# mgokbulut/CG-RayTracer

Hardware: NVIDIA B200
Metric: Mrays/s (primary+shadow+bounce) (higher is better)
Workload: dtype f32

## Files before the change

cg-raytracer_b200/csrc/cgrt_capi.cu:

```cuda
#include "../../include/cgrt_b200.h"
#include "bvh_build.h"
#include "cgrt_kernels.h"

#include <algorithm>
#include <cfloat>
#include <climits>
#include <cmath>
#include <cstdio>
#include <cstring>
#include <map>
#include <mutex>
#include <string>
#include <vector>

using namespace cgrt;
#ifdef CGRT_INSTRUMENT
namespace cgrt { void readInstrumentation(unsigned long long* out, bool reset); void readTimeline(unsigned int* out, bool reset); void readStepHist(unsigned int* out, bool reset); }
#endif

static thread_local std::string g_err;
static int fail(int code, const std::string& msg)
{
    g_err = msg;
    return code;
// ... 1080 lines not shown
    T.recording = -1;
}

static bool waveTuning(WaveQ& Q, int nSlots, int nLights, int world)
{
    static int mode = 0, groupBelow = 400000, fin = 0, timeoutMs = 4000, switchBelow = 0, handOver = 1, tune = 1;
    static bool loaded = false;
    if (!loaded) {
        loaded = true;
        if (const char* e = getenv("CGRT_WAVE")) {
            std::string t(e);
            size_t pos = 0;
            while (pos < t.size()) {
                size_t c = t.find(',', pos);
                if (c == std::string::npos) c = t.size();
                const std::string kv = t.substr(pos, c - pos);
                const size_t eq = kv.find('=');
                if (eq != std::string::npos) {
                    const std::string key = kv.substr(0, eq);
                    const int v = atoi(kv.c_str() + eq + 1);
                    if (key == "mode") mode = v;
                    else if (key == "group_below") groupBelow = v;
                    else if (key == "fin") fin = v;
                    else if (key == "switch") switchBelow = v;
                    else if (key == "timeout_ms") timeoutMs = v;
                    else if (key == "handover") handOver = v;
                    else if (key == "tune") tune = v;
                }
                pos = c + 1;
            }
        }
    }
    Q.mode = mode == 1 || mode == 2 ? mode : (nSlots < groupBelow ? 2 : 1);
    Q.finEvery = fin > 0 ? std::max(fin, 2) : (nLights >= 3 ? 4 : (nLights == 2 ? 5 : (Q.mode == 2 && world > 1 ? 8 : 6)));
    Q.switchBelow = Q.mode == 2 ? 0 : (switchBelow > 0 ? switchBelow : (nSlots >= 1500000 ? 100000 : 60000));
    Q.timeoutNs = (unsigned long long)std::max(timeoutMs, 1) * 1000000ull;
    if (!handOver) Q.resume = nullptr;
    return fin <= 0 && tune != 0;
}

static int prepareFrame(cgrt_scene* s, const cgrt_camera* cams, int nViews, const cgrt_render_params* p, FrameParams& P,
                        const int** dTileList, const int2** dTileSeq, FramePipeline* pipe)
{
    const int tw = p->tile_w > 0 ? p->tile_w : 8, th = p->tile_h > 0 ? p->tile_h : 8;
    const int key[6] = {p->width, p->height, tw, th, p->world, p->rank};
    if (std::memcmp(key, s->tileKey, sizeof key) != 0 || !s->tileSeq.p) {
        TileLayout& L = s->layout;
        makeTileLayout(*p, L);
        const std::vector<int>& mine = L.lists[p->rank];
        std::vector<int2> seq(mine.size());
        std::vector<std::pair<float, int>> order(mine.size());
        s->primaryPixels = 0;
        for (size_t lt = 0; lt < mine.size(); lt++) {
            const int ty = mine[lt] / L.tilesX, tx = mine[lt] % L.tilesX;
            const float cx = (tx + 0.5f) * L.tileW - 0.5f * p->width, cy = (ty + 0.5f) * L.tileH - 0.5f * p->height;
            order[lt] = std::make_pair(cx * cx + cy * cy, (int)lt);
            const int w = std::min(L.tileW, p->width - tx * L.tileW), h = std::min(L.tileH, p->height - ty * L.tileH);
            s->primaryPixels += (uint64_t)w * h;
        }
        std::sort(order.begin(), order.end());
        for (size_t k = 0; k < order.size(); k++) seq[k] = make_int2(mine[order[k].second], order[k].second);
        RC(s->tileList.ensure(std::max<size_t>(mine.size(), 1)));
        RC(s->tileSeq.ensure(std::max<size_t>(mine.size(), 1)));
        CK(cudaDeviceSynchronize());
        if (!mine.empty()) {
            CK(cudaMemcpy(s->tileList.p, mine.data(), mine.size() * sizeof(int), cudaMemcpyHostToDevice));
            CK(cudaMemcpy(s->tileSeq.p, seq.data(), seq.size() * sizeof(int2), cudaMemcpyHostToDevice));
// ... 15 lines not shown
    P.tilesX = L.tilesX;
    P.world = L.world;
    P.rank = p->rank;
    P.screenLayout = (L.world == 1 || (p->flags & CGRT_RENDER_SCREEN_LAYOUT)) ? 1 : 0;
    const int64_t slots = (int64_t)nViews * (int64_t)L.lists[p->rank].size() * L.tileW * L.tileH;
    if (slots > INT_MAX) return fail(CGRT_ERR_INVALID, "too many pixel slots: views x tiles x tile pixels must stay below 2^31");
    P.nSlots = (int)slots;
    *dTileList = L.world > 1 ? s->tileList.p : nullptr;
    *dTileSeq = s->tileSeq.p;
    const size_t cap = (size_t)std::max(P.nSlots, 1);
    const int nL = std::max(P.nLights, 1);
    const int levels = std::max(P.traceLimit - 1, 1);
    const int pathLevels = std::max(P.traceLimit, 1);
    if (P.nSph > 0 && !useRounds(s, P)) return fail(CGRT_ERR_INVALID, "spherical lights need a scene with a search tree (not CGRT_SCENE_EXACT_ONLY / NO_SUBTREES)");
    *pipe = choosePipeline(s, P, p->flags);
    if (*pipe != PIPE_COUNT) {
        RC(s->hitRec.ensure(cap * pathLevels * 3));
        RC(s->pathDepth.ensure(cap));
        RC(s->lit.ensure(cap * pathLevels * nL));
    }
    switch (*pipe) {
    case PIPE_COUNT:
        RC(s->hitQ.ensure(cap * 3));
        RC(s->bounceQ.ensure(cap * 2));
        RC(s->lit.ensure(cap * nL));
        RC(s->pathState.ensure(cap * 2 * levels));
        break;
    case PIPE_WAVE: {
        const size_t tickets = waveTicketCap(P);
        if (tickets >= ((size_t)1 << 30)) return fail(CGRT_ERR_INVALID, "frame too large for the ray queue's 30-bit tickets");
        if (!s->waveRays.p || s->waveRays.n < tickets * 3) {
            RC(s->waveRays.ensure(tickets * 3));
            CK(cudaMemset(s->waveRays.p, 0, tickets * 3 * sizeof(float4)));
            RC(s->waveFin.ensure(tickets * 2));
            CK(cudaMemset(s->waveFin.p, 0, tickets * 2 * sizeof(float4)));
            CK(uploadsDone());
        }
        RC(s->waveCtl.ensure(WCTL_INTS));
        RC(s->waveResume.ensure((size_t)waveGridBlocks(s->di.numSMs) * 128 * WAVE_RESUME_F4));
        break;
    }
    case PIPE_ROUNDS: {
        if (P.nSph > 0) {
            RC(s->softList.ensure(cap * pathLevels + 1));
            RC(s->soft.ensure(cap * pathLevels * (size_t)P.nSph));
        }
        const size_t capR = cap + (size_t)CGRT_MAX_CHAINS * P.tileW * P.tileH;
        for (int k = 0; k < 2; k++) {
            RC(s->cRay[k].ensure(capR * 3));
            RC(s->cRes[k].ensure(capR));
            RC(s->sRay[k].ensure(capR * nL * 3));
            RC(s->sRes[k].ensure(capR * nL));
        }
        break;
    }
    case PIPE_PATHS:
        RC(s->hitList.ensure(cap * pathLevels));
        if (s->dev.fastRoot != 0u) {
            RC(s->replayQ.ensure(cap * 3));
            RC(s->replayShadow.ensure(cap * pathLevels * nL));
        }
        break;
    }
    RC(s->pathPix.ensure(cap));
    RC(s->counts.ensure(CGRT_CNT_TOTAL * CGRT_MAX_CHAINS));
    RC(s->tests.ensure(6));
    const size_t need = CGRT_PARAM_BLOCK_HEADER + ((size_t)nL + (size_t)P.nSph) * 32 + (size_t)nViews * CGRT_VIEW_F4 * 16;
    if (need > s->paramBlockBytes || !s->hParamRing) {
// ... 41 lines not shown
    B.replayQ = s->replayQ.p;
    B.replayShadow = s->replayShadow.p;
    B.counts = s->counts.p;
    B.cap = (size_t)std::max(P.nSlots, 1);
    B.levels = std::max(P.traceLimit, 1);
    return B;
}

static RoundBuffers roundBuffers(const cgrt_scene* s, const FrameParams& P, int c, int nChains)
{
    const size_t tpx = (size_t)P.tileW * P.tileH;
    const size_t capC = ((size_t)std::max(P.nSlots, 1) / tpx / nChains + 1) * tpx;
    const size_t nLc = (size_t)std::max(P.nLights, 1);
    RoundBuffers B;
    for (int k = 0; k < 2; k++) {
        B.cRay[k] = s->cRay[k].p + c * capC * 3; B.cRes[k] = s->cRes[k].p + c * capC;
        B.sRay[k] = s->sRay[k].p + c * capC * nLc * 3; B.sRes[k] = s->sRes[k].p + c * capC * nLc;
    }
    B.hitRec = s->hitRec.p;
    B.lit = s->lit.p;
    B.pathDepth = s->pathDepth.p;
    B.counts = s->counts.p + c * CGRT_CNT_TOTAL;
    B.levels = std::max(P.traceLimit, 1);
    B.softList = s->softList.p;
    B.soft = s->soft.p;
    B.softSeed = s->softSeed;
    return B;
}

static int waveQueues(cgrt_scene* s, cudaStream_t st, WaveQ& Q)
{
    Q.rays = s->waveRays.p;
    Q.fin = s->waveFin.p;
    Q.ctl = s->waveCtl.p;
    Q.seq = ++s->waveSeq;
    if (Q.seq == 0u) Q.seq = ++s->waveSeq;
    Q.cap = (int)std::min<size_t>(s->waveRays.n / 3, (size_t)0x3fffffff);
    Q.resume = s->waveResume.p;
    Q.resumeCap = (int)std::min<size_t>(s->waveResume.n / WAVE_RESUME_F4, (size_t)0xffffff);
    Q.lat = nullptr;
#ifdef CGRT_WAVE_LAT
    if (getenv("CGRT_WAVE_LAT")) {
        RC(s->waveLat.ensure((size_t)Q.cap * 16));
        CK(cudaMemsetAsync(s->waveLat.p, 0, (size_t)Q.cap * 16 * sizeof(unsigned), st));
        Q.lat = s->waveLat.p;
    }
#endif
    Q.trace = nullptr;
    if (getenv("CGRT_WAVE_TRACE") || Q.lat != nullptr) {
        RC(s->waveTrace.ensure((size_t)WAVE_TRACE_SAMPLES * 8));
        CK(cudaMemsetAsync(s->waveTrace.p, 0, (size_t)WAVE_TRACE_SAMPLES * 8 * sizeof(int), st));
        Q.trace = s->waveTrace.p;
    }
    return CGRT_OK;
}

static int renderDevice(cgrt_scene* s, const cgrt_camera* cams, int nViews, const cgrt_render_params* p, float* d_out, void* stream)
{
    RC(useSceneDevice(s));
    std::lock_guard<std::mutex> lk(s->mu);
    cudaStream_t st = (cudaStream_t)stream;
    FrameParams P;
    const int* dTiles = nullptr;
    const int2* dSeq = nullptr;
    FramePipeline pipe;
    RC(prepareFrame(s, cams, nViews, p, P, &dTiles, &dSeq, &pipe));
// ... 659 lines not shown
```

cg-raytracer_b200/csrc/cgrt_kernels.h:

```cpp
#pragma once
#include <cuda_runtime.h>
#include <stdint.h>
#include <stddef.h>

struct DevScene {
    const float4* nodes;
    const float4* triPl;
    const float4* triV0;
    const float4* triV1;
    const float4* triV2;
    const float4* tri4;
    const float4* tri4f;
    const float4* triN0;
    const float4* triN1;
    const float4* triN2;
    const float4* mats;
    const float4* spheres;
    const float4* pairs;
    const float4* wide;
    const float4* wide8;
    const int* origToLeaf;
    const int* alwaysTri;
    int nAlways;
    const int* refParent;
// ... 66 lines not shown
    int levels;
};

struct RoundBuffers {
    float4* cRay[2];
    float4* cRes[2];
    float4* sRay[2];
    float4* sRes[2];
    float4* hitRec;
    uint8_t* lit;
    int* pathDepth;
    int* counts;
    int levels;
    int* softList;
    float* soft;
    unsigned softSeed;
};

#define WCTL_PENDING 0
#define WCTL_ERR 2
#define WCTL_HEAD 32
#define WCTL_TAIL 64
#define WCTL_FHEAD 96
#define WCTL_FTAIL 128
#define WCTL_HEAD2 160
#define WCTL_TAIL2 192
#define WCTL_FINCOUNT 288
#define WCTL_FINEXIT 289
#define WCTL_T0 4
#define WCTL_CLOSEAT 224
#define WCTL_RESUME 256
#define WCTL_DONE 320
#define WCTL_SCRATCH (WCTL_DONE + 32 * 32)
#define WCTL_INTS (WCTL_SCRATCH + 32 * 32)

struct WaveQ {
    float4* rays;
    float4* fin;
    int* ctl;
    uint32_t seq;
    int cap;
    int mode;
    int switchBelow;
    int finEvery;
    unsigned long long timeoutNs;
    int resumeCap;
    float4* resume;
    unsigned* lat;
    int* trace;
};
#define WAVE_TRACE_SAMPLES 1024
#define WAVE_RESUME_STACK 32
#define WAVE_RESUME_F4 (1 + WAVE_RESUME_STACK / 2)

#define CGRT_TRACE_MAX_KERNELS (8 * (2 * (CGRT_MAX_LEVELS + 1) + 1) + 2)
struct WaveTrace {
    cudaEvent_t* ev;
    int maxKernels;
    int classMask;
    int n;
    int cls[CGRT_TRACE_MAX_KERNELS];
    int launches[4];
};

void launchSetupPlanes(const float4* v0, const float4* v1, const float4* v2, float4* pl, float4* tri4, int n, cudaStream_t st);
void launchPermuteTri4(const float4* tri4, const int* fastOrder, float4* tri4f, int n, cudaStream_t st);
void launchClosestBatch(const DevScene& S, const float4* rays, size_t n, float4* hits, uint32_t* counts, int numSMs,
                        cudaStream_t st);
void launchAnyBatch(const DevScene& S, const float4* rays, const float* maxDist, float eps, size_t n, uint8_t* occluded,
                    int numSMs, cudaStream_t st);
void launchBruteBatch(const DevScene& S, const float4* rays, size_t n, float4* hits, int numSMs, cudaStream_t st);
// ... 38 lines not shown
```

cg-raytracer_b200/csrc/cgrt_wave.cuh:

```cuda
#pragma once

#define WAVE_NSTAT 40
#define WAVE_STAT_PATHS 0
#define WAVE_STAT_HIT 1
#define WAVE_STAT_BOUNCE 17
#define WAVE_STAT_REPLAYC 35
#define WAVE_STAT_REPLAYS 36
struct WaveShared {
    int stat[WAVE_NSTAT];
    uint2 gstack[16][CGRT_STACK8];
};

enum { WS_NONE = 0, WS_WAIT = 1, WS_RUN = 2, WS_PASS = 3 };

RT_DEV unsigned ldRelaxedGpu(const unsigned* p)
{
    unsigned v;
    asm volatile("ld.relaxed.gpu.global.u32 %0, [%1];" : "=r"(v) : "l"(p) : "memory");
    return v;
}
RT_DEV void stRelaxedGpu(unsigned* p, unsigned v) { asm volatile("st.relaxed.gpu.global.u32 [%0], %1;" ::"l"(p), "r"(v) : "memory"); }
RT_DEV float4 ld128(const float4* p)
{
    unsigned long long lo, hi;
    asm volatile("{ .reg .b128 t; ld.relaxed.gpu.global.b128 t, [%2]; mov.b128 {%0, %1}, t; }" : "=l"(lo), "=l"(hi) : "l"(p) : "memory");
    return make_float4(__uint_as_float((unsigned)lo), __uint_as_float((unsigned)(lo >> 32)), __uint_as_float((unsigned)hi),
                       __uint_as_float((unsigned)(hi >> 32)));
}
RT_DEV void st128(float4* p, const float4& v)
{
    const unsigned long long lo = (unsigned long long)__float_as_uint(v.x) | ((unsigned long long)__float_as_uint(v.y) << 32);
    const unsigned long long hi = (unsigned long long)__float_as_uint(v.z) | ((unsigned long long)__float_as_uint(v.w) << 32);
    asm volatile("{ .reg .b128 t; mov.b128 t, {%1, %2}; st.relaxed.gpu.global.b128 [%0], t; }" ::"l"(p), "l"(lo), "l"(hi) : "memory");
}
RT_DEV void waveRelease(const WaveQ& Q)
{
    int* scratch = Q.ctl + WCTL_SCRATCH + 32 * ((blockIdx.x * 4 + (threadIdx.x >> 5)) & 31);
    asm volatile("red.release.gpu.global.add.u32 [%0], %1;" ::"l"(scratch), "r"(0) : "memory");
}
RT_DEV unsigned long long globalTimerNs()
{
    unsigned long long t;
    asm volatile("mov.u64 %0, %%globaltimer;" : "=l"(t));
    return t;
}
RT_DEV unsigned smId()
{
    unsigned v;
    asm("mov.u32 %0, %%smid;" : "=r"(v));
    return v;
}

#ifdef CGRT_WAVE_LAT
RT_DEV void waveLat(const WaveQ& Q, int tk, int k, unsigned v)
{
    if (Q.lat != nullptr && tk >= 0 && tk < Q.cap) Q.lat[16 * (size_t)tk + k] = v;
}
RT_DEV unsigned waveNow(const WaveQ& Q) { return (unsigned)globalTimerNs() - ldRelaxedGpu((const unsigned*)Q.ctl + WCTL_T0); }
#define WAVE_LAT(tk, k, v) waveLat(Q, tk, k, v)
#define WAVE_LAT_NOW(tk, k) waveLat(Q, tk, k, waveNow(Q))
#else
#define WAVE_LAT(tk, k, v)
#define WAVE_LAT_NOW(tk, k)
#endif

#define WAVE_SLOT_BITS 26
#define WAVE_CLOSED 0x40000000
#define WAVE_TAG2 0x80000000u
RT_DEV void waveStoreRay(const WaveQ& Q, int tk, unsigned tagBits, const V3& o, const V3& d, float bound, int meta)
{
    if (tk >= Q.cap) return;
    float4* q = Q.rays + 3 * (size_t)tk;
    const float tag = __uint_as_float(tagBits);
    st128(q, make_float4(o.x, o.y, o.z, tag));
    st128(q + 1, make_float4(d.x, d.y, d.z, tag));
    st128(q + 2, make_float4(bound, i2f(meta), 0.0f, tag));
    WAVE_LAT_NOW(tk, 0);
}
RT_DEV bool waveLoadRay(const WaveQ& Q, int tk, unsigned tagBits, float4& a, float4& b, float4& c)
{
    if (tk >= Q.cap) return false;
    const float4* r = Q.rays + 3 * (size_t)tk;
    a = ld128(r);
    b = ld128(r + 1);
    const float4 m = ld128(r + 2);
    const unsigned s = tagBits;
    const bool ok = __float_as_uint(a.w) == s && __float_as_uint(b.w) == s && __float_as_uint(m.w) == s;
    const int meta = f2i(m.y);
    if (meta & CGRT_RAY_ANY) {
        a.w = FLT_MAX;
        b.w = m.x;
        c = make_float4(0.0f, m.y, 0.001f, m.z);
    } else {
        a.w = m.x;
        b.w = __int_as_float(0x7f800000);
        c = make_float4(i2f(meta & ((1 << WAVE_SLOT_BITS) - 1)), i2f(meta >> WAVE_SLOT_BITS), 0.0f, m.z);
    }
    return ok;
}
RT_DEV bool wavePeekRay(const WaveQ& Q, bool mine, int tk, unsigned tagBits)
{
    const unsigned m = __ballot_sync(0xffffffffu, mine);
    if (m == 0u) return false;
    const int lowest = __reduce_min_sync(0xffffffffu, mine ? tk : 0x7fffffff);
    unsigned w = 0u;
    if ((threadIdx.x & 31) == 0 && lowest < Q.cap) w = ldRelaxedGpu((const unsigned*)(Q.rays + 3 * (size_t)lowest) + 11);
    return __shfl_sync(0xffffffffu, w, 0) == tagBits;
}
RT_DEV bool wavePeekFin(const WaveQ& Q, bool mine, int ftk)
{
    const unsigned m = __ballot_sync(0xffffffffu, mine);
    if (m == 0u) return false;
    const int lowest = __reduce_min_sync(0xffffffffu, mine ? ftk : 0x7fffffff);
    unsigned w = 0u;
    if ((threadIdx.x & 31) == 0 && lowest < Q.cap) w = ldRelaxedGpu((const unsigned*)(Q.fin + 2 * (size_t)lowest) + 7);
    return __shfl_sync(0xffffffffu, w, 0) == Q.seq;
}
RT_DEV int waveReserve(const WaveQ& Q, int n, bool& closedSeen, unsigned& tagBits)
{
    if (!closedSeen) {
        const int old = atomicAdd(Q.ctl + WCTL_TAIL, n);
        if (!(old & WAVE_CLOSED)) {
            tagBits = Q.seq;
            return old;
        }
        closedSeen = true;
    }
    const int t2 = atomicAdd(Q.ctl + WCTL_TAIL2, n);
    unsigned ca;
    while ((ca = ldRelaxedGpu((const unsigned*)Q.ctl + WCTL_CLOSEAT)) == 0u) { }
    tagBits = Q.seq | WAVE_TAG2;
    return (int)(ca - 1u) + t2;
}
RT_DEV int waveClaim(const WaveQ& Q, int headIdx, int n)
{
    int base = 0;
    if ((threadIdx.x & 31) == 0) base = atomicAdd(Q.ctl + headIdx, n);
    return __shfl_sync(0xffffffffu, base, 0);
}
RT_DEV void waveFinPush(const WaveQ& Q, bool mine, int tk, int state, float t, int tri, float t2)
{
    const unsigned mask = __ballot_sync(0xffffffffu, mine);
    if (mask == 0u) return;
    const int lane = threadIdx.x & 31, leader = __ffs(mask) - 1;
    int base = 0;
    if (lane == leader) base = atomicAdd(Q.ctl + WCTL_FTAIL, __popc(mask));
    base = __shfl_sync(0xffffffffu, base, leader);
    if (mine) {
        const int pos = base + __popc(mask & ((1u << lane) - 1u));
        if (pos < Q.cap) {
            const float tag = __uint_as_float(Q.seq);
            st128(Q.fin + 2 * (size_t)pos, make_float4(i2f(tk), i2f(state), t, tag));
            st128(Q.fin + 2 * (size_t)pos + 1, make_float4(i2f(tri), t2, tag, tag));
        }
    }
}
RT_DEV bool waveLoadFin(const WaveQ& Q, int ftk, int& tk, float4& res)
{
    if (ftk >= Q.cap) return false;
    const float4 c0 = ld128(Q.fin + 2 * (size_t)ftk), c1 = ld128(Q.fin + 2 * (size_t)ftk + 1);
    const unsigned s = Q.seq;
    tk = f2i(c0.x);
    res = make_float4(c0.y, c0.z, c1.x, c1.y);
    return __float_as_uint(c0.w) == s && __float_as_uint(c1.z) == s && __float_as_uint(c1.w) == s;
}
RT_DEV void waveRaiseDone(const WaveQ& Q)
{
    waveRelease(Q);
#pragma unroll 1
    for (int k = 0; k < 32; k++) stRelaxedGpu((unsigned*)Q.ctl + WCTL_DONE + 32 * k, 1u);
}
RT_DEV void wavePending(const WaveQ& Q, long long delta)
{
    unsigned long long* pend = (unsigned long long*)Q.ctl;
    const unsigned long long now = atomicAdd(pend, (unsigned long long)delta) + (unsigned long long)delta;
    if (now == ((unsigned long long)gridDim.x << 32)) {
        waveRaiseDone(Q);
    } else if (delta < 0 && Q.switchBelow > 0 && (now >> 32) == (unsigned long long)gridDim.x && (unsigned)now < (unsigned)Q.switchBelow) {
        if (ldRelaxedGpu((const unsigned*)Q.ctl + WCTL_CLOSEAT) == 0u) {
            const int old = atomicOr(Q.ctl + WCTL_TAIL, WAVE_CLOSED);
            if (!(old & WAVE_CLOSED)) stRelaxedGpu((unsigned*)Q.ctl + WCTL_CLOSEAT, (unsigned)old + 1u);
        }
    }
}
RT_DEV void wavePendingAdd(const WaveQ& Q, int created) { atomicAdd((unsigned long long*)Q.ctl, (unsigned long long)created); }
RT_DEV unsigned long long wavePendingIssue(const WaveQ& Q, long long delta)
{
    return atomicAdd((unsigned long long*)Q.ctl, (unsigned long long)delta) + (unsigned long long)delta;
}
RT_DEV void wavePendingCheck(const WaveQ& Q, unsigned long long now)
{
    if (now == ((unsigned long long)gridDim.x << 32)) {
        waveRaiseDone(Q);
// ... 4 lines not shown
        }
    }
}
RT_DEV bool waveDone(const WaveQ& Q)
{
    const int w = (blockIdx.x * 4 + (threadIdx.x >> 5)) & 31;
    unsigned f = 0u;
    if ((threadIdx.x & 31) == 0) f = ldRelaxedGpu((const unsigned*)Q.ctl + WCTL_DONE + 32 * w);
    return __shfl_sync(0xffffffffu, f, 0) != 0u;
}
#ifndef CGRT_WAVE_IDLE_MAX
#define CGRT_WAVE_IDLE_MAX 1000
#endif
RT_DEV void waveIdle(const WaveQ& Q, unsigned long long t0, int& idlePolls)
{
    __nanosleep(idlePolls < 8 ? 100 : (idlePolls < 32 ? 250 : (idlePolls < 128 ? 500 : CGRT_WAVE_IDLE_MAX)));
    if ((++idlePolls & 63) == 0 && (threadIdx.x & 31) == 0 && globalTimerNs() - t0 > Q.timeoutNs) {
        atomicExch(Q.ctl + WCTL_ERR, 1);
        waveRaiseDone(Q);
    }
}

RT_DEV void waveTraceSample(const WaveQ& Q, int& lastBucket)
{
    if (Q.trace == nullptr || (blockIdx.x & 15) != 0 || (threadIdx.x & 127) != 0) return;
    const unsigned t0 = ldRelaxedGpu((const unsigned*)Q.ctl + WCTL_T0);
    const int bucket = (int)(((unsigned)globalTimerNs() - t0) >> 12);
    if (bucket == lastBucket || bucket < 0 || bucket >= WAVE_TRACE_SAMPLES) return;
    lastBucket = bucket;
    int* o = Q.trace + 8 * bucket;
    o[1] = (int)ldRelaxedGpu((const unsigned*)Q.ctl + WCTL_PENDING);
    o[2] = (int)ldRelaxedGpu((const unsigned*)Q.ctl + WCTL_HEAD);
    o[3] = (int)ldRelaxedGpu((const unsigned*)Q.ctl + WCTL_TAIL);
    o[4] = (int)ldRelaxedGpu((const unsigned*)Q.ctl + WCTL_FHEAD);
    o[5] = (int)ldRelaxedGpu((const unsigned*)Q.ctl + WCTL_FTAIL);
    o[6] = (int)ldRelaxedGpu((const unsigned*)Q.ctl + WCTL_HEAD2);
    o[7] = (int)ldRelaxedGpu((const unsigned*)Q.ctl + WCTL_TAIL2);
    o[0] = 1;
}

#ifndef CGRT_WAVE_FIN_WAIT
#define CGRT_WAVE_FIN_WAIT 3
#endif
RT_DEV void waveFinishLoop(const DevScene& S, const FrameParams& P, const float4* __restrict__ lights, const WaveQ& Q,
                           const RoundBuffers& B, const int2* __restrict__ tileSeq, float* __restrict__ fb, WaveShared& sh,
                           unsigned long long t0)
{
    const int lane = threadIdx.x & 31;
    const unsigned ltMask = (1u << lane) - 1u;
    const int nL = P.nLights;
    int ftk = -1;
    int waited = 0, idlePolls = 0;
    bool closedSeen = false;
    int traceBucket = -1;
    int nextBase = 0, nextCount = 0;
    unsigned long long pendNow = 0ull;
    bool havePend = false, busy = false;
    {
        const int base = waveClaim(Q, WCTL_FHEAD, 32);
        ftk = base + lane;
    }
    while (true) {
        waveTraceSample(Q, traceBucket);
        if (nextCount) {
            const unsigned noneMask = __ballot_sync(0xffffffffu, ftk < 0);
            const int base = __shfl_sync(0xffffffffu, nextBase, 0);
            if (ftk < 0) ftk = base + __popc(noneMask & ltMask);
            nextCount = 0;
        }
        int tk = -1;
        float4 res = make_float4(0.0f, 0.0f, 0.0f, 0.0f);
        const bool ready = (busy || waited > 0 || wavePeekFin(Q, true, ftk)) && waveLoadFin(Q, ftk, tk, res);
        if (havePend) {
            wavePendingCheck(Q, pendNow);
            havePend = false;
        }
        const unsigned readyMask = __ballot_sync(0xffffffffu, ready);
        if (readyMask == 0u) {
            busy = false;
            if (waveDone(Q)) break;
            waveIdle(Q, t0, idlePolls);
            continue;
        }
        idlePolls = 0;
        if (readyMask != 0xffffffffu && busy && ++waited < CGRT_WAVE_FIN_WAIT) continue;
        busy = readyMask == 0xffffffffu && waited == 0;
        waited = 0;
        nextCount = __popc(readyMask);
        if (lane == 0) nextBase = atomicAdd(Q.ctl + WCTL_FHEAD, nextCount);
        const int n = __popc(readyMask);
        bool hit = false, bounce = false, replayC = false, replayS = false;
        V3 pointOn = mk3(0.0f, 0.0f, 0.0f), nn = pointOn, rd = pointOn;
        int slot = 0, rec = 0, level = 0;
        if (ready) {
            ftk = -1;
            float4 a, b, c;
            WAVE_LAT_NOW(tk, 4);
            waveLoadRay(Q, tk, 0u, a, b, c);
            const int meta = f2i(c.y);
#ifdef CGRT_WAVE_LAT
            if (a.x == 1e38f) return;
            WAVE_LAT_NOW(tk, 8);
#endif
            if (meta & CGRT_RAY_ANY) {
                const bool shadowed = finishShadowRay<true>(S, a, b, c, res, replayS);
                WAVE_LAT_NOW(tk, 9);
                B.lit[meta & 0x3fffffff] = shadowed ? 0 : 1;
            } else {
                const V3 o = mk3(a), d = mk3(b);
                slot = f2i(c.x);
                level = meta;
                TraceResult R;
                hit = finishClosestRay<true>(S, a, b, res, R, replayC);
#ifdef CGRT_WAVE_LAT
                if (R.t == -1e38f) return;
                WAVE_LAT_NOW(tk, 9);
#endif
                if (!hit) {
                    if (level == 0) {
                        int x, y, outIdx, local;
                        if (seqToPixel(P, tileSeq, slot, x, y, outIdx, local)) storeRGB(fb, outIdx, mk3(0.0f, 0.0f, 0.0f));
                    }
                } else {
                    int mat;
                    hitNormalAndMaterial(S, R, o, d, nn, mat);
                    pointOn = o + d * R.t;
                    rd = d;
                    rec = slot * B.levels + level;
                    float4* h = B.hitRec + 3 * (size_t)rec;
                    h[0] = make_float4(pointOn.x, pointOn.y, pointOn.z, i2f(mat));
                    h[1] = make_float4(nn.x, nn.y, nn.z, 0.0f);
                    h[2] = make_float4(d.x, d.y, d.z, 0.0f);
                    B.pathDepth[slot] = level + 1;
                    const float ksz = mat >= 0 ? __ldg(S.mats + 2 * mat + 1).z : 0.0f;
                    bounce = !(ksz <= 0.01f) && level + 1 < P.traceLimit;
                    atomicAdd(&sh.stat[WAVE_STAT_HIT + level], 1);
                    if (level == 0) atomicAdd(&sh.stat[WAVE_STAT_PATHS], 1);
                    if (bounce) atomicAdd(&sh.stat[WAVE_STAT_BOUNCE + level + 1], 1);
                    WAVE_LAT_NOW(tk, 10);
                }
                if (replayC) atomicAdd(&sh.stat[WAVE_STAT_REPLAYC], 1);
            }
            if (replayS) atomicAdd(&sh.stat[WAVE_STAT_REPLAYS], 1);
        }
        const int nShadow = hit ? nL : 0, nBounce = bounce ? 1 : 0;
        int sIncl = nShadow, bIncl = nBounce;
#pragma unroll
        for (int o = 1; o < 32; o <<= 1) {
            const int vs = __shfl_up_sync(0xffffffffu, sIncl, o), vb = __shfl_up_sync(0xffffffffu, bIncl, o);
            if (lane >= o) { sIncl += vs; bIncl += vb; }
        }
        const int totS = __shfl_sync(0xffffffffu, sIncl, 31), totB = __shfl_sync(0xffffffffu, bIncl, 31);
        int base = 0;
        unsigned tagBits = 0u;
        if (lane == 0 && totS + totB > 0) {
            wavePendingAdd(Q, totS + totB);
            base = waveReserve(Q, totS + totB, closedSeen, tagBits);
        }
        base = __shfl_sync(0xffffffffu, base, 0);
        tagBits = __shfl_sync(0xffffffffu, tagBits, 0);
        if (ready) WAVE_LAT_NOW(tk, 11);
        if (hit && nL > 0) {
            const int firstS = base + sIncl - nShadow;
            for (int l = 0; l < nL; l++) {
                V3 org, dir;
                float dist;
                shadowRayOf(lights, l, pointOn, org, dir, dist);
                waveStoreRay(Q, firstS + l, tagBits, org, dir, dist, CGRT_RAY_ANY | (rec * nL + l));
            }
        }
        if (bounce) {
            V3 org, dir;
            float tIn;
            reflectionRayOf(pointOn, rd, nn, org, dir, tIn);
            waveStoreRay(Q, base + totS + bIncl - 1, tagBits, org, dir, tIn, ((level + 1) << WAVE_SLOT_BITS) | slot);
        }
        if (ready) WAVE_LAT_NOW(tk, 5);
        if (lane == 0) {
            pendNow = wavePendingIssue(Q, -(long long)n);
            havePend = true;
        }
    }
    waveRelease(Q);
    __syncwarp();
    if (lane == 0) atomicAdd(Q.ctl + WCTL_FINEXIT, 1);
}

#ifndef CGRT_WAVE_STEPS
#define CGRT_WAVE_STEPS 8
#endif
#ifndef CGRT_WAVE_REFILL
#define CGRT_WAVE_REFILL 16
#endif
#ifndef CGRT_WAVE_GFIN
#define CGRT_WAVE_GFIN 1
#endif
#ifndef CGRT_WAVE_GSTEPS
#define CGRT_WAVE_GSTEPS 8
#endif
RT_DEV bool waveLaneLoop(const DevScene& S, const WaveQ& Q, unsigned long long t0)
{
    const int lane = threadIdx.x & 31;
    const unsigned ltMask = (1u << lane) - 1u;
    FastTrav T;
    FastStack K;
    int tk = -1, st = WS_NONE, state = TRAV_DONE;
    float eps = 0.0f, maxDist = 0.0f;
    bool any = false;
    int idlePolls = 0;
    int closeAt = 0x7fffffff;
    bool drained = false;
    T.t = 0.0f; T.hitTri = -1; T.node = 0u; T.sp = 0;
    K.t2 = 0.0f;
    while (true) {
        const bool fin = st == WS_RUN && state != TRAV_CONTINUE;
        const unsigned finMask = __ballot_sync(0xffffffffu, fin);
        const unsigned runMask = __ballot_sync(0xffffffffu, st == WS_RUN && !fin);
        const unsigned waitMask = __ballot_sync(0xffffffffu, st == WS_WAIT);
        const unsigned noneMask = __ballot_sync(0xffffffffu, st == WS_NONE || fin);
        const int nNone = __popc(noneMask), nFin = __popc(finMask);
        const bool open = closeAt == 0x7fffffff;
        const int want = (!drained && (!open || nNone >= CGRT_WAVE_REFILL || runMask == 0u) && nNone > 0) ? nNone : 0;
        int fbase = 0, base = 0;
        unsigned ca = 0u;
        if (lane == 0) {
            if (nFin) fbase = atomicAdd(Q.ctl + WCTL_FTAIL, nFin);
            if (want) base = atomicAdd(Q.ctl + WCTL_HEAD, want);
            if (open && Q.switchBelow > 0 && (waitMask != 0u || want != 0)) ca = ldRelaxedGpu((const unsigned*)Q.ctl + WCTL_CLOSEAT);
        }
        if (nFin) {
            fbase = __shfl_sync(0xffffffffu, fbase, 0);
            if (fin) {
                const int pos = fbase + __popc(finMask & ltMask);
                if (pos < Q.cap) {
                    const float tag = __uint_as_float(Q.seq);
                    st128(Q.fin + 2 * (size_t)pos, make_float4(i2f(tk), i2f(state), T.t, tag));
                    st128(Q.fin + 2 * (size_t)pos + 1, make_float4(i2f(T.hitTri), K.t2, tag, tag));
                }
                WAVE_LAT_NOW(tk, 3);
                st = WS_NONE;
                tk = -1;
            }
        }
        if (want) {
            base = __shfl_sync(0xffffffffu, base, 0);
            if (st == WS_NONE) {
                tk = base + __popc(noneMask & ltMask);
                st = WS_WAIT;
            }
        }
        if (open && Q.switchBelow > 0) {
            ca = __shfl_sync(0xffffffffu, ca, 0);
            if (ca != 0u) closeAt = (int)(ca - 1u);
        }
        const bool closed = closeAt != 0x7fffffff;
        if (closed && want != 0 && base + want > closeAt) drained = true;
        if (st == WS_WAIT && tk >= closeAt) { st = WS_NONE; tk = -1; }
        const bool handOver = closed && Q.resume != nullptr;
        if (handOver) {
            const bool mig = st == WS_RUN && state == TRAV_CONTINUE && T.sp <= WAVE_RESUME_STACK;
            const unsigned migMask = __ballot_sync(0xffffffffu, mig);
            if (migMask != 0u) {
                int rbase = 0, qbase = 0;
                if (lane == 0) {
                    rbase = atomicAdd(Q.ctl + WCTL_RESUME, __popc(migMask));
                    qbase = atomicAdd(Q.ctl + WCTL_TAIL2, __popc(migMask));
                }
                rbase = __shfl_sync(0xffffffffu, rbase, 0);
                qbase = __shfl_sync(0xffffffffu, qbase, 0);
                if (mig) {
                    const int r = rbase + __popc(migMask & ltMask), ntk = closeAt + qbase + __popc(migMask & ltMask);
// ... 69 lines not shown
            const bool run = st == WS_RUN && state == TRAV_CONTINUE;
            const bool leaf = run && travIsLeaf(T.node);
            const int sAll = __popc(__ballot_sync(0xffffffffu, run));
            const int sLeaf = __popc(__ballot_sync(0xffffffffu, leaf));
            const int nDone = __popc(__ballot_sync(0xffffffffu, st == WS_RUN && state != TRAV_CONTINUE));
            if (sAll == 0 || (nDone >= CGRT_WAVE_REFILL && it > 0)) break;
            if (sAll - sLeaf >= sLeaf) {
                if (run && !leaf) state = fastStepWideDyn(S, T, K, any, maxDist);
            } else {
                if (leaf) state = fastStepLeafDyn(S, T, K, any, eps, maxDist);
            }
        }
    }
}

RT_DEV void waveGroupLoop(const DevScene& S, const WaveQ& Q, WaveShared& sh, unsigned long long t0, int headIdx, int baseIdx,
                          unsigned tagBits)
{
    const int lane = threadIdx.x & 31, g = lane >> 3, j = lane & 7;
    uint2* K = sh.gstack[threadIdx.x >> 3];
    const float slack = 1.000001f;
    V3 o = mk3(0.0f, 0.0f, 0.0f), d = o, inv = o;
    float t = 0.0f, t2 = 0.0f, eps = 0.0f, maxDist = 0.0f;
    int hitTri = -1, tk = -1, st = WS_NONE, state = TRAV_DONE, sp = 0;
    uint32_t node = 0u;
    bool any = false;
    int idlePolls = 0;
#ifdef CGRT_WAVE_LAT
    int nsteps = 0;
#endif
    while (true) {
        const bool fin = st == WS_RUN && state != TRAV_CONTINUE;
        if (__any_sync(0xffffffffu, fin)) {
            waveFinPush(Q, fin && j == 0, tk, state, t, hitTri, t2);
#ifdef CGRT_WAVE_LAT
            if (fin && j == 0) { WAVE_LAT_NOW(tk, 3); WAVE_LAT(tk, 2, (unsigned)nsteps); }
#endif
            if (fin) { st = WS_NONE; tk = -1; }
        }
        const unsigned needy = __ballot_sync(0xffffffffu, st == WS_NONE && j == 0);
        if (needy != 0u) {
            const int base = waveClaim(Q, headIdx, __popc(needy));
            if (st == WS_NONE) {
                tk = baseIdx + base + __popc(needy & ((1u << (8 * g)) - 1u));
                st = WS_WAIT;
            }
        }
        const bool anyRun = __ballot_sync(0xffffffffu, st == WS_RUN) != 0u;
        if (anyRun ? __any_sync(0xffffffffu, st == WS_WAIT) : wavePeekRay(Q, st == WS_WAIT, tk, tagBits)) {
            float4 a = make_float4(0.0f, 0.0f, 0.0f, 0.0f), b = a, c = a;
            const bool rdy = st == WS_WAIT && waveLoadRay(Q, tk, tagBits, a, b, c);
            const unsigned rm = __ballot_sync(0xffffffffu, rdy);
            const bool start = ((rm >> (8 * g)) & 0xFFu) == 0xFFu;
            if (start) {
                o = mk3(a);
                d = mk3(b);
                maxDist = b.w;
                eps = c.z;
                any = (f2i(c.y) & CGRT_RAY_ANY) != 0;
                FastTrav T0;
                state = fastBegin(S, T0, o, d, a.w);
                inv = T0.inv;
                t = T0.t;
                t2 = __int_as_float(0x7f800000);
                hitTri = T0.hitTri;
                sp = 0;
                node = T0.node;
// ... 282 lines not shown
```

Before: 2641.

## Split wave finish queue into separate closest-hit and shadow queues

Finished traversal records now go into two queues, one for closest-hit rays and one for shadow (any-hit) rays, each with its own head and tail counters. A single 64-bit atomic reserves slots in both at once. The finisher warps consume homogeneous batches from one queue at a time, so shadow and closest-hit shading no longer diverge within a warp. The change also alters the default finEvery for mode 1 with one light, and doubles the finish-buffer size.

```diff
diff --git a/cg-raytracer_b200/csrc/cgrt_capi.cu b/cg-raytracer_b200/csrc/cgrt_capi.cu
--- a/cg-raytracer_b200/csrc/cgrt_capi.cu
+++ b/cg-raytracer_b200/csrc/cgrt_capi.cu
@@ -1136,7 +1136,7 @@
         }
     }
     Q.mode = mode == 1 || mode == 2 ? mode : (nSlots < groupBelow ? 2 : 1);
-    Q.finEvery = fin > 0 ? std::max(fin, 2) : (nLights >= 3 ? 4 : (nLights == 2 ? 5 : (Q.mode == 2 && world > 1 ? 8 : 6)));
+    Q.finEvery = fin > 0 ? std::max(fin, 2) : (nLights >= 3 ? 4 : (nLights == 2 ? 5 : (Q.mode == 2 ? (world > 1 ? 8 : 6) : 7)));
     Q.switchBelow = Q.mode == 2 ? 0 : (switchBelow > 0 ? switchBelow : (nSlots >= 1500000 ? 100000 : 60000));
     Q.timeoutNs = (unsigned long long)std::max(timeoutMs, 1) * 1000000ull;
     if (!handOver) Q.resume = nullptr;
@@ -1218,8 +1218,8 @@
         if (!s->waveRays.p || s->waveRays.n < tickets * 3) {
             RC(s->waveRays.ensure(tickets * 3));
             CK(cudaMemset(s->waveRays.p, 0, tickets * 3 * sizeof(float4)));
-            RC(s->waveFin.ensure(tickets * 2));
-            CK(cudaMemset(s->waveFin.p, 0, tickets * 2 * sizeof(float4)));
+            RC(s->waveFin.ensure(tickets * 4));
+            CK(cudaMemset(s->waveFin.p, 0, tickets * 4 * sizeof(float4)));
             CK(uploadsDone());
         }
         RC(s->waveCtl.ensure(WCTL_INTS));
@@ -1327,6 +1327,7 @@
 {
     Q.rays = s->waveRays.p;
     Q.fin = s->waveFin.p;
+    Q.sfin = s->waveFin.p + s->waveFin.n / 2;
     Q.ctl = s->waveCtl.p;
     Q.seq = ++s->waveSeq;
     if (Q.seq == 0u) Q.seq = ++s->waveSeq;
diff --git a/cg-raytracer_b200/csrc/cgrt_kernels.h b/cg-raytracer_b200/csrc/cgrt_kernels.h
--- a/cg-raytracer_b200/csrc/cgrt_kernels.h
+++ b/cg-raytracer_b200/csrc/cgrt_kernels.h
@@ -122,11 +122,14 @@
 #define WCTL_RESUME 256
 #define WCTL_DONE 320
 #define WCTL_SCRATCH (WCTL_DONE + 32 * 32)
-#define WCTL_INTS (WCTL_SCRATCH + 32 * 32)
+#define WCTL_SFHEAD (WCTL_SCRATCH + 32 * 32)
+#define WCTL_SFTAIL (WCTL_FTAIL + 1)
+#define WCTL_INTS (WCTL_SFHEAD + 32)
 
 struct WaveQ {
     float4* rays;
     float4* fin;
+    float4* sfin;
     int* ctl;
     uint32_t seq;
     int cap;
diff --git a/cg-raytracer_b200/csrc/cgrt_wave.cuh b/cg-raytracer_b200/csrc/cgrt_wave.cuh
--- a/cg-raytracer_b200/csrc/cgrt_wave.cuh
+++ b/cg-raytracer_b200/csrc/cgrt_wave.cuh
@@ -52,6 +52,11 @@
 }
 
 #ifdef CGRT_WAVE_LAT
+#define WAVE_LAT_CLOSEST_HIT 1u
+#define WAVE_LAT_CLOSEST_MISS 2u
+#define WAVE_LAT_SHADOW_FIRED 3u
+#define WAVE_LAT_SHADOW_DONE 4u
+#define WAVE_LAT_REPLAY 8u
 RT_DEV void waveLat(const WaveQ& Q, int tk, int k, unsigned v)
 {
     if (Q.lat != nullptr && tk >= 0 && tk < Q.cap) Q.lat[16 * (size_t)tk + k] = v;
@@ -107,14 +112,16 @@
     if ((threadIdx.x & 31) == 0 && lowest < Q.cap) w = ldRelaxedGpu((const unsigned*)(Q.rays + 3 * (size_t)lowest) + 11);
     return __shfl_sync(0xffffffffu, w, 0) == tagBits;
 }
-RT_DEV bool wavePeekFin(const WaveQ& Q, bool mine, int ftk)
-{
-    const unsigned m = __ballot_sync(0xffffffffu, mine);
-    if (m == 0u) return false;
-    const int lowest = __reduce_min_sync(0xffffffffu, mine ? ftk : 0x7fffffff);
-    unsigned w = 0u;
-    if ((threadIdx.x & 31) == 0 && lowest < Q.cap) w = ldRelaxedGpu((const unsigned*)(Q.fin + 2 * (size_t)lowest) + 7);
-    return __shfl_sync(0xffffffffu, w, 0) == Q.seq;
+RT_DEV void wavePeekFin(const WaveQ& Q, int ftkC, int ftkS, bool& servedC, bool& servedS)
+{
+    const int lowC = __reduce_min_sync(0xffffffffu, ftkC), lowS = __reduce_min_sync(0xffffffffu, ftkS);
+    unsigned wc = 0u, ws = 0u;
+    if ((threadIdx.x & 31) == 0) {
+        if (lowC < Q.cap) wc = ldRelaxedGpu((const unsigned*)(Q.fin + 2 * (size_t)lowC) + 7);
+        if (lowS < Q.cap) ws = ldRelaxedGpu((const unsigned*)(Q.sfin + 2 * (size_t)lowS) + 7);
+    }
+    servedC = __shfl_sync(0xffffffffu, wc, 0) == Q.seq;
+    servedS = __shfl_sync(0xffffffffu, ws, 0) == Q.seq;
 }
 RT_DEV int waveReserve(const WaveQ& Q, int n, bool& closedSeen, unsigned& tagBits)
 {
@@ -138,27 +145,34 @@
     if ((threadIdx.x & 31) == 0) base = atomicAdd(Q.ctl + headIdx, n);
     return __shfl_sync(0xffffffffu, base, 0);
 }
-RT_DEV void waveFinPush(const WaveQ& Q, bool mine, int tk, int state, float t, int tri, float t2)
+RT_DEV void waveFinStore(const WaveQ& Q, bool any, int pos, int tk, int state, float t, int tri, float t2)
+{
+    if (pos >= Q.cap) return;
+    float4* f = (any ? Q.sfin : Q.fin) + 2 * (size_t)pos;
+    const float tag = __uint_as_float(Q.seq);
+    st128(f, make_float4(i2f(tk), i2f(state), t, tag));
+    st128(f + 1, make_float4(i2f(tri), t2, tag, tag));
+}
+RT_DEV unsigned long long waveFinReserve(const WaveQ& Q, unsigned cMask, unsigned sMask)
+{
+    return atomicAdd((unsigned long long*)(Q.ctl + WCTL_FTAIL), (unsigned long long)__popc(cMask) | ((unsigned long long)__popc(sMask) << 32));
+}
+RT_DEV void waveFinPush(const WaveQ& Q, bool mine, bool any, int tk, int state, float t, int tri, float t2)
 {
     const unsigned mask = __ballot_sync(0xffffffffu, mine);
     if (mask == 0u) return;
+    const unsigned sMask = __ballot_sync(0xffffffffu, mine && any), cMask = mask & ~sMask;
     const int lane = threadIdx.x & 31, leader = __ffs(mask) - 1;
-    int base = 0;
-    if (lane == leader) base = atomicAdd(Q.ctl + WCTL_FTAIL, __popc(mask));
-    base = __shfl_sync(0xffffffffu, base, leader);
-    if (mine) {
-        const int pos = base + __popc(mask & ((1u << lane) - 1u));
-        if (pos < Q.cap) {
-            const float tag = __uint_as_float(Q.seq);
-            st128(Q.fin + 2 * (size_t)pos, make_float4(i2f(tk), i2f(state), t, tag));
-            st128(Q.fin + 2 * (size_t)pos + 1, make_float4(i2f(tri), t2, tag, tag));
-        }
-    }
-}
-RT_DEV bool waveLoadFin(const WaveQ& Q, int ftk, int& tk, float4& res)
+    unsigned long long bases = 0ull;
+    if (lane == leader) bases = waveFinReserve(Q, cMask, sMask);
+    bases = __shfl_sync(0xffffffffu, bases, leader);
+    if (mine) waveFinStore(Q, any, (int)(any ? (unsigned)(bases >> 32) : (unsigned)bases) + __popc((any ? sMask : cMask) & ((1u << lane) - 1u)), tk, state, t, tri, t2);
+}
+RT_DEV bool waveLoadFin(const WaveQ& Q, bool any, int ftk, int& tk, float4& res)
 {
     if (ftk >= Q.cap) return false;
-    const float4 c0 = ld128(Q.fin + 2 * (size_t)ftk), c1 = ld128(Q.fin + 2 * (size_t)ftk + 1);
+    const float4* f = (any ? Q.sfin : Q.fin) + 2 * (size_t)ftk;
+    const float4 c0 = ld128(f), c1 = ld128(f + 1);
     const unsigned s = Q.seq;
     tk = f2i(c0.x);
     res = make_float4(c0.y, c0.z, c1.x, c1.y);
@@ -229,8 +243,8 @@
     o[1] = (int)ldRelaxedGpu((const unsigned*)Q.ctl + WCTL_PENDING);
     o[2] = (int)ldRelaxedGpu((const unsigned*)Q.ctl + WCTL_HEAD);
     o[3] = (int)ldRelaxedGpu((const unsigned*)Q.ctl + WCTL_TAIL);
-    o[4] = (int)ldRelaxedGpu((const unsigned*)Q.ctl + WCTL_FHEAD);
-    o[5] = (int)ldRelaxedGpu((const unsigned*)Q.ctl + WCTL_FTAIL);
+    o[4] = (int)(ldRelaxedGpu((const unsigned*)Q.ctl + WCTL_FHEAD) + ldRelaxedGpu((const unsigned*)Q.ctl + WCTL_SFHEAD));
+    o[5] = (int)(ldRelaxedGpu((const unsigned*)Q.ctl + WCTL_FTAIL) + ldRelaxedGpu((const unsigned*)Q.ctl + WCTL_SFTAIL));
     o[6] = (int)ldRelaxedGpu((const unsigned*)Q.ctl + WCTL_HEAD2);
     o[7] = (int)ldRelaxedGpu((const unsigned*)Q.ctl + WCTL_TAIL2);
     o[0] = 1;
@@ -246,72 +260,124 @@
     const int lane = threadIdx.x & 31;
     const unsigned ltMask = (1u << lane) - 1u;
     const int nL = P.nLights;
-    int ftk = -1;
-    int waited = 0, idlePolls = 0;
+    int ftkC = -1, ftkS = -1;
+    int waitedC = 0, waitedS = 0, idlePolls = 0;
     bool closedSeen = false;
     int traceBucket = -1;
     int nextBase = 0, nextCount = 0;
+    bool lastShadow = false;
     unsigned long long pendNow = 0ull;
-    bool havePend = false, busy = false;
+    bool havePend = false, busyC = false, busyS = false;
     {
-        const int base = waveClaim(Q, WCTL_FHEAD, 32);
-        ftk = base + lane;
+        int baseC = 0, baseS = 0;
+        if (lane == 0) {
+            baseC = atomicAdd(Q.ctl + WCTL_FHEAD, 32);
+            baseS = atomicAdd(Q.ctl + WCTL_SFHEAD, 32);
+        }
+        ftkC = __shfl_sync(0xffffffffu, baseC, 0) + lane;
+        ftkS = __shfl_sync(0xffffffffu, baseS, 0) + lane;
     }
     while (true) {
         waveTraceSample(Q, traceBucket);
         if (nextCount) {
-            const unsigned noneMask = __ballot_sync(0xffffffffu, ftk < 0);
+            const bool none = (lastShadow ? ftkS : ftkC) < 0;
+            const unsigned noneMask = __ballot_sync(0xffffffffu, none);
             const int base = __shfl_sync(0xffffffffu, nextBase, 0);
-            if (ftk < 0) ftk = base + __popc(noneMask & ltMask);
+            if (none) {
+                if (lastShadow) ftkS = base + __popc(noneMask & ltMask);
+                else ftkC = base + __popc(noneMask & ltMask);
+            }
             nextCount = 0;
         }
-        int tk = -1;
-        float4 res = make_float4(0.0f, 0.0f, 0.0f, 0.0f);
-        const bool ready = (busy || waited > 0 || wavePeekFin(Q, true, ftk)) && waveLoadFin(Q, ftk, tk, res);
+        bool lookC = busyC || waitedC > 0, lookS = busyS || waitedS > 0;
+        if (!lookC || !lookS) {
+            bool servedC, servedS;
+            wavePeekFin(Q, ftkC, ftkS, servedC, servedS);
+            lookC = lookC || servedC;
+            lookS = lookS || servedS;
+        }
+        int tkC = -1, tkS = -1;
+        float4 resC = make_float4(0.0f, 0.0f, 0.0f, 0.0f), resS = resC;
+        const bool readyC = lookC && waveLoadFin(Q, false, ftkC, tkC, resC);
+        const bool readyS = lookS && waveLoadFin(Q, true, ftkS, tkS, resS);
         if (havePend) {
             wavePendingCheck(Q, pendNow);
             havePend = false;
         }
-        const unsigned readyMask = __ballot_sync(0xffffffffu, ready);
-        if (readyMask == 0u) {
-            busy = false;
+        const unsigned maskC = __ballot_sync(0xffffffffu, readyC), maskS = __ballot_sync(0xffffffffu, readyS);
+        if (maskC == 0u) busyC = false;
+        if (maskS == 0u) busyS = false;
+        if ((maskC | maskS) == 0u) {
             if (waveDone(Q)) break;
             waveIdle(Q, t0, idlePolls);
             continue;
         }
         idlePolls = 0;
-        if (readyMask != 0xffffffffu && busy && ++waited < CGRT_WAVE_FIN_WAIT) continue;
-        busy = readyMask == 0xffffffffu && waited == 0;
-        waited = 0;
+        const bool goC = maskC != 0u && (maskC == 0xffffffffu || !busyC || ++waitedC >= CGRT_WAVE_FIN_WAIT);
+        const bool goS = maskS != 0u && (maskS == 0xffffffffu || !busyS || ++waitedS >= CGRT_WAVE_FIN_WAIT);
+        if (!goC && !goS) continue;
+        const bool shadowBatch = goS && !goC;
+        lastShadow = shadowBatch;
+        const unsigned readyMask = shadowBatch ? maskS : maskC;
+        if (shadowBatch) {
+            busyS = maskS == 0xffffffffu && waitedS == 0;
+            waitedS = 0;
+        } else {
+            busyC = maskC == 0xffffffffu && waitedC == 0;
+            waitedC = 0;
+        }
         nextCount = __popc(readyMask);
-        if (lane == 0) nextBase = atomicAdd(Q.ctl + WCTL_FHEAD, nextCount);
-        const int n = __popc(readyMask);
-        bool hit = false, bounce = false, replayC = false, replayS = false;
-        V3 pointOn = mk3(0.0f, 0.0f, 0.0f), nn = pointOn, rd = pointOn;
-        int slot = 0, rec = 0, level = 0;
-        if (ready) {
-            ftk = -1;
-            float4 a, b, c;
-            WAVE_LAT_NOW(tk, 4);
-            waveLoadRay(Q, tk, 0u, a, b, c);
-            const int meta = f2i(c.y);
-#ifdef CGRT_WAVE_LAT
-            if (a.x == 1e38f) return;
-            WAVE_LAT_NOW(tk, 8);
-#endif
-            if (meta & CGRT_RAY_ANY) {
-                const bool shadowed = finishShadowRay<true>(S, a, b, c, res, replayS);
-                WAVE_LAT_NOW(tk, 9);
+        if (lane == 0) nextBase = atomicAdd(Q.ctl + (shadowBatch ? WCTL_SFHEAD : WCTL_FHEAD), nextCount);
+        const int n = nextCount;
+#ifdef CGRT_WAVE_LAT
+        const unsigned latB0 = __shfl_sync(0xffffffffu, waveNow(Q), 0);
+        unsigned latCls = 0u;
+        const int tk = shadowBatch ? tkS : tkC;
+        const bool ready = shadowBatch ? readyS : readyC;
+#endif
+        if (shadowBatch) {
+            if (readyS) {
+                ftkS = -1;
+                float4 a, b, c;
+                bool replayS = false;
+                WAVE_LAT_NOW(tkS, 4);
+                waveLoadRay(Q, tkS, 0u, a, b, c);
+                const int meta = f2i(c.y);
+#ifdef CGRT_WAVE_LAT
+                if (a.x == 1e38f) return;
+                WAVE_LAT_NOW(tkS, 8);
+#endif
+                const bool shadowed = finishShadowRay<true>(S, a, b, c, resS, replayS);
+                WAVE_LAT_NOW(tkS, 9);
                 B.lit[meta & 0x3fffffff] = shadowed ? 0 : 1;
-            } else {
+#ifdef CGRT_WAVE_LAT
+                latCls = (f2i(resS.x) == TRAV_FIRED ? WAVE_LAT_SHADOW_FIRED : WAVE_LAT_SHADOW_DONE) | (replayS ? WAVE_LAT_REPLAY : 0u);
+#endif
+                if (replayS) atomicAdd(&sh.stat[WAVE_STAT_REPLAYS], 1);
+                WAVE_LAT_NOW(tkS, 11);
+                WAVE_LAT_NOW(tkS, 5);
+            }
+        } else {
+            bool hit = false, bounce = false, replayC = false;
+            V3 pointOn = mk3(0.0f, 0.0f, 0.0f), nn = pointOn, rd = pointOn;
+            int slot = 0, rec = 0, level = 0;
+            if (readyC) {
+                ftkC = -1;
+                float4 a, b, c;
+                WAVE_LAT_NOW(tkC, 4);
+                waveLoadRay(Q, tkC, 0u, a, b, c);
+#ifdef CGRT_WAVE_LAT
+                if (a.x == 1e38f) return;
+                WAVE_LAT_NOW(tkC, 8);
+#endif
                 const V3 o = mk3(a), d = mk3(b);
                 slot = f2i(c.x);
-                level = meta;
+                level = f2i(c.y);
                 TraceResult R;
-                hit = finishClosestRay<true>(S, a, b, res, R, replayC);
+                hit = finishClosestRay<true>(S, a, b, resC, R, replayC);
 #ifdef CGRT_WAVE_LAT
                 if (R.t == -1e38f) return;
-                WAVE_LAT_NOW(tk, 9);
+                WAVE_LAT_NOW(tkC, 9);
 #endif
                 if (!hit) {
                     if (level == 0) {
@@ -334,45 +400,51 @@
                     atomicAdd(&sh.stat[WAVE_STAT_HIT + level], 1);
                     if (level == 0) atomicAdd(&sh.stat[WAVE_STAT_PATHS], 1);
                     if (bounce) atomicAdd(&sh.stat[WAVE_STAT_BOUNCE + level + 1], 1);
-                    WAVE_LAT_NOW(tk, 10);
+                    WAVE_LAT_NOW(tkC, 10);
                 }
                 if (replayC) atomicAdd(&sh.stat[WAVE_STAT_REPLAYC], 1);
-            }
-            if (replayS) atomicAdd(&sh.stat[WAVE_STAT_REPLAYS], 1);
-        }
-        const int nShadow = hit ? nL : 0, nBounce = bounce ? 1 : 0;
-        int sIncl = nShadow, bIncl = nBounce;
+#ifdef CGRT_WAVE_LAT
+                latCls = (hit ? WAVE_LAT_CLOSEST_HIT : WAVE_LAT_CLOSEST_MISS) | (replayC ? WAVE_LAT_REPLAY : 0u);
+#endif
+            }
+            const int nShadow = hit ? nL : 0, nBounce = bounce ? 1 : 0;
+            int sIncl = nShadow, bIncl = nBounce;
 #pragma unroll
-        for (int o = 1; o < 32; o <<= 1) {
-            const int vs = __shfl_up_sync(0xffffffffu, sIncl, o), vb = __shfl_up_sync(0xffffffffu, bIncl, o);
-            if (lane >= o) { sIncl += vs; bIncl += vb; }
-        }
-        const int totS = __shfl_sync(0xffffffffu, sIncl, 31), totB = __shfl_sync(0xffffffffu, bIncl, 31);
-        int base = 0;
-        unsigned tagBits = 0u;
-        if (lane == 0 && totS + totB > 0) {
-            wavePendingAdd(Q, totS + totB);
-            base = waveReserve(Q, totS + totB, closedSeen, tagBits);
-        }
-        base = __shfl_sync(0xffffffffu, base, 0);
-        tagBits = __shfl_sync(0xffffffffu, tagBits, 0);
-        if (ready) WAVE_LAT_NOW(tk, 11);
-        if (hit && nL > 0) {
-            const int firstS = base + sIncl - nShadow;
-            for (int l = 0; l < nL; l++) {
+            for (int o = 1; o < 32; o <<= 1) {
+                const int vs = __shfl_up_sync(0xffffffffu, sIncl, o), vb = __shfl_up_sync(0xffffffffu, bIncl, o);
+                if (lane >= o) { sIncl += vs; bIncl += vb; }
+            }
+            const int totS = __shfl_sync(0xffffffffu, sIncl, 31), totB = __shfl_sync(0xffffffffu, bIncl, 31);
+            int base = 0;
+            unsigned tagBits = 0u;
+            if (lane == 0 && totS + totB > 0) {
+                wavePendingAdd(Q, totS + totB);
+                base = waveReserve(Q, totS + totB, closedSeen, tagBits);
+            }
+            base = __shfl_sync(0xffffffffu, base, 0);
+            tagBits = __shfl_sync(0xffffffffu, tagBits, 0);
+            if (readyC) WAVE_LAT_NOW(tkC, 11);
+            if (hit && nL > 0) {
+                const int firstS = base + sIncl - nShadow;
+                for (int l = 0; l < nL; l++) {
+                    V3 org, dir;
+                    float dist;
+                    shadowRayOf(lights, l, pointOn, org, dir, dist);
+                    waveStoreRay(Q, firstS + l, tagBits, org, dir, dist, CGRT_RAY_ANY | (rec * nL + l));
+                }
+            }
+            if (bounce) {
                 V3 org, dir;
-                float dist;
-                shadowRayOf(lights, l, pointOn, org, dir, dist);
-                waveStoreRay(Q, firstS + l, tagBits, org, dir, dist, CGRT_RAY_ANY | (rec * nL + l));
-            }
-        }
-        if (bounce) {
-            V3 org, dir;
-            float tIn;
-            reflectionRayOf(pointOn, rd, nn, org, dir, tIn);
-            waveStoreRay(Q, base + totS + bIncl - 1, tagBits, org, dir, tIn, ((level + 1) << WAVE_SLOT_BITS) | slot);
-        }
-        if (ready) WAVE_LAT_NOW(tk, 5);
+                float tIn;
+                reflectionRayOf(pointOn, rd, nn, org, dir, tIn);
+                waveStoreRay(Q, base + totS + bIncl - 1, tagBits, org, dir, tIn, ((level + 1) << WAVE_SLOT_BITS) | slot);
+            }
+            if (readyC) WAVE_LAT_NOW(tkC, 5);
+        }
+#ifdef CGRT_WAVE_LAT
+        const unsigned latB1 = __shfl_sync(0xffffffffu, waveNow(Q), 0);
+        if (ready) { WAVE_LAT(tk, 12, latB0); WAVE_LAT(tk, 13, latB1); WAVE_LAT(tk, 14, 1u + blockIdx.x * 4 + (threadIdx.x >> 5)); WAVE_LAT(tk, 15, latCls); }
+#endif
         if (lane == 0) {
             pendNow = wavePendingIssue(Q, -(long long)n);
             havePend = true;
@@ -412,28 +484,25 @@
     while (true) {
         const bool fin = st == WS_RUN && state != TRAV_CONTINUE;
         const unsigned finMask = __ballot_sync(0xffffffffu, fin);
+        const unsigned sfinMask = __ballot_sync(0xffffffffu, fin && any), cfinMask = finMask & ~sfinMask;
         const unsigned runMask = __ballot_sync(0xffffffffu, st == WS_RUN && !fin);
         const unsigned waitMask = __ballot_sync(0xffffffffu, st == WS_WAIT);
         const unsigned noneMask = __ballot_sync(0xffffffffu, st == WS_NONE || fin);
         const int nNone = __popc(noneMask), nFin = __popc(finMask);
         const bool open = closeAt == 0x7fffffff;
         const int want = (!drained && (!open || nNone >= CGRT_WAVE_REFILL || runMask == 0u) && nNone > 0) ? nNone : 0;
-        int fbase = 0, base = 0;
+        unsigned long long fbase = 0ull;
+        int base = 0;
         unsigned ca = 0u;
         if (lane == 0) {
-            if (nFin) fbase = atomicAdd(Q.ctl + WCTL_FTAIL, nFin);
+            if (nFin) fbase = waveFinReserve(Q, cfinMask, sfinMask);
             if (want) base = atomicAdd(Q.ctl + WCTL_HEAD, want);
             if (open && Q.switchBelow > 0 && (waitMask != 0u || want != 0)) ca = ldRelaxedGpu((const unsigned*)Q.ctl + WCTL_CLOSEAT);
         }
         if (nFin) {
             fbase = __shfl_sync(0xffffffffu, fbase, 0);
             if (fin) {
-                const int pos = fbase + __popc(finMask & ltMask);
-                if (pos < Q.cap) {
-                    const float tag = __uint_as_float(Q.seq);
-                    st128(Q.fin + 2 * (size_t)pos, make_float4(i2f(tk), i2f(state), T.t, tag));
-                    st128(Q.fin + 2 * (size_t)pos + 1, make_float4(i2f(T.hitTri), K.t2, tag, tag));
-                }
+                waveFinStore(Q, any, (int)(any ? (unsigned)(fbase >> 32) : (unsigned)fbase) + __popc((any ? sfinMask : cfinMask) & ltMask), tk, state, T.t, T.hitTri, K.t2);
                 WAVE_LAT_NOW(tk, 3);
                 st = WS_NONE;
                 tk = -1;
@@ -569,7 +638,7 @@
     while (true) {
         const bool fin = st == WS_RUN && state != TRAV_CONTINUE;
         if (__any_sync(0xffffffffu, fin)) {
-            waveFinPush(Q, fin && j == 0, tk, state, t, hitTri, t2);
+            waveFinPush(Q, fin && j == 0, any, tk, state, t, hitTri, t2);
 #ifdef CGRT_WAVE_LAT
             if (fin && j == 0) { WAVE_LAT_NOW(tk, 3); WAVE_LAT(tk, 2, (unsigned)nsteps); }
 #endif
```

New measurement: 2690, median of 6. +1.9%, better.
